# NVlabs/L4P

Measured on AMD Instinct MI355X. Metric: frames/sec (all heads), 16x224x224 clip; encoder MFMA-roofline %, higher is better.
Workload: dtype bf16; 1 GPU; configs[2]: single MI355X, all heads (depth+flow+track2d/3d+motion-seg+pose), bf16, batch=4 clips, 64 track queries per clip; parallelism=dp1 (clips sharded, no collective in the step)

## Files before the change

### l4p_amd/csrc/gemm8p.hpp

```cpp
#pragma once
#include "gemm.hpp"

#ifdef GEMM_PROBE_VARIANTS
static __device__ int g_tile_gm = 0;
#endif
template <int WR, int WC, int TM, int TN>
struct Gemm8pCfg {
    static constexpr int BM = WR * TM * 16, BN = WC * TN * 16;
    static constexpr int A_HALF = WR * TM * 8 * 128, W_HALF = (WC * TN * 8 + 63) / 64 * 64 * 128;
    static constexpr int LDS_BYTES = 2 * (2 * A_HALF + 2 * W_HALF);
};
template <typename T, int MODE, int WR, int WC, bool SPLITK = false, int TM = 8, int TN = 4, bool PERSIST = false, bool SUBPIX = false>
__global__ __launch_bounds__(512) void gemm8p_kernel(const GemmParams p) {
    static_assert(!PERSIST || (MODE == 0 && !SPLITK), "persistent form: dense GEMM without split-K");
    static_assert(!SUBPIX || (MODE == 1 && !SPLITK && !PERSIST), "sub-pixel conv: the conv form without split-K");
    static_assert(WR * WC == 8 && (WC == 2 || WC == 4), "8 waves");
    static_assert(TM % 2 == 0 && TN % 2 == 0 && (WR * TM) % 8 == 0, "half tiles; A half-tile = whole 64-row staging passes");
    constexpr int BM = WR * TM * 16, BN = WC * TN * 16, BK = 64;
    constexpr int RH = TM * 8, CH = TN * 8;
    constexpr int A_PASS = WR * RH / 64, W_PASS = (WC * CH + 63) / 64;
    constexpr int A_HALF = WR * RH * 128, W_HALF = W_PASS * 64 * 128;
    constexpr int BUF = 2 * A_HALF + 2 * W_HALF;
    constexpr int INFLIGHT = 2 * A_PASS + 2 * W_PASS;
    typedef const __attribute__((address_space(1))) void* gptr_t;
    typedef __attribute__((address_space(3))) void* lptr_t;

    extern __shared__ __attribute__((aligned(16))) char smem[];

    const int wave = __builtin_amdgcn_readfirstlane((int)threadIdx.x >> 6);
    const int wr = wave / WC, wc = wave % WC, grp = wave >> 2;
    int li, kg, srow, slot, cs_a, cs_w[W_PASS], a_off[2], w_off[2];
    auto lane_setup = [&](int tid) {
        const int lane = tid & 63;
        li = lane & 15, kg = lane >> 4;
        srow = tid >> 3, slot = tid & 7;
        cs_a = slot ^ ((srow >> 1) & 7);
#pragma unroll
        for (int i = 0; i < W_PASS; ++i) {
            const int lr = srow + 64 * i;
            cs_w[i] = slot ^ (((((lr % CH) / (2 * TN)) & 3) << 1) | ((lr >> 1) & 1));
        }
        const int sw_a = (li >> 1) & 7, sw_w = (((li >> 2) & 3) << 1) | ((li >> 1) & 1);
#pragma unroll
        for (int kk = 0; kk < 2; ++kk) {
            a_off[kk] = (wr * RH + li) * 128 + (((kk * 4 + kg) ^ sw_a) << 4);
            w_off[kk] = (wc * CH + 2 * TN * (li >> 2) + (li & 3)) * 128 + (((kk * 4 + kg) ^ sw_w) << 4);
        }
    };
    lane_setup((int)threadIdx.x);

    const int ntn = (p.N + BN - 1) / BN, ntm = (p.M + BM - 1) / BM, ntiles = ntn * ntm;
    const int nsplit = SPLITK ? p.splitk : 1;
    const int ksplit = SPLITK ? (int)blockIdx.x / ntiles : 0;
    const int bid0 = SPLITK ? (int)blockIdx.x - ksplit * ntiles : (int)blockIdx.x;
    auto decode_tile = [&](int bid, int& m0_, int& n0_) {
        int tile;
        {
            const int xcd = bid & 7, idx = bid >> 3, q = ntiles >> 3, r = ntiles & 7;
            tile = (xcd < r ? xcd * (q + 1) : r * (q + 1) + (xcd - r) * q) + idx;
        }
        int mt, nt_;
        {
            const int nb = (ntn + 7) >> 3, bw = (ntn + nb - 1) / nb, full = (nb - 1) * ntm * bw;
#ifdef GEMM_PROBE_VARIANTS
            const bool banded = g_tile_gm >= 0;
#else
            const bool banded = true;
#endif
            if (!banded || nb == 1) {
                mt = tile / ntn;
                nt_ = tile % ntn;
            } else if (tile < full) {
                const int band = tile / (ntm * bw), rem = tile - band * (ntm * bw);
                mt = rem / bw;
                nt_ = band * bw + rem % bw;
            } else {
                const int w = ntn - (nb - 1) * bw, rem = tile - full;
                mt = rem / w;
                nt_ = (nb - 1) * bw + rem % w;
            }
        }
        if (MODE == 1) mt = conv_tile_walk(p, mt, BM, 2);
        m0_ = mt * BM, n0_ = nt_ * BN;
    };
    int bid = bid0, m0, n0;
    decode_tile(bid, m0, n0);

    const char* a_src[A_PASS][2];
    unsigned a_mask[A_PASS][2];
    const char* w_src[W_PASS][2];
    auto setup_src = [&](int m0, int n0) {
#pragma unroll
    for (int i = 0; i < A_PASS; ++i)
#pragma unroll
        for (int h = 0; h < 2; ++h) {
            const int lra = i * 64 + srow;
            int m = m0 + (lra / RH) * (TM * 16) + h * RH + lra % RH;
// ... 43 lines not shown
    const int kt0 = SPLITK ? (int)((long long)nk_all * ksplit / nsplit) : 0;
    const int nk = SPLITK ? (int)((long long)nk_all * (ksplit + 1) / nsplit) - kt0 : nk_all;
    const char* zero = (const char*)g_zero_chunk;

    struct ConvPos {
        int kt, tap, ci0;
        long long off;
        int bit;
    } cpos[2];
    auto conv_tap_off = [&](int tap) {
        const int dt = tap / 9 - 1, dh = (tap / 3) % 3 - 1, dw = tap % 3 - 1;
        return ((((long long)dt * p.Hi + dh) * p.Wi + dw) * p.Cin) * 2;
    };
    if (MODE == 1) {
#pragma unroll
        for (int h = 0; h < 2; ++h) {
            const int first = SUBPIX ? subpix_tap(cells, 0) : 0;
            cpos[h] = ConvPos{0, 0, 0, conv_tap_off(first), first};
        }
    }
    auto stage_a = [&](int h, int kt, int buf) {
        long long off;
        int tap = 0;
        if (MODE == 0) {
            off = (long long)(kt0 + kt) * (BK * 2);
        } else {
            ConvPos& c = cpos[h];
            while (c.kt < kt0 + kt) {
                ++c.kt;
                c.ci0 += BK;
                if (c.ci0 == p.Cin) {
                    c.ci0 = 0;
                    ++c.tap;
                    if constexpr (SUBPIX) {
                        c.bit = subpix_tap(cells, c.tap);
                        c.off = conv_tap_off(c.bit);
                    } else {
                        c.off = conv_tap_off(c.tap < 27 ? c.tap : 26);
                    }
                }
            }
            tap = SUBPIX ? c.bit : c.tap;
            off = c.off + (long long)c.ci0 * 2;
        }
#pragma unroll
        for (int i = 0; i < A_PASS; ++i) {
            bool ok;
            if (MODE == 0)
                ok = (!SPLITK || kt < nk) && (kt0 + kt) * BK + cs_a * 8 < p.K;
            else
                ok = kt < nk && ((a_mask[i][h] >> tap) & 1u);
            const char* src = ok ? a_src[i][h] + off : zero;
            __builtin_amdgcn_global_load_lds((gptr_t)src, (lptr_t)(smem + buf * BUF + h * A_HALF + (i * 512 + wave * 64) * 16), 16,
                                             0, 0);
        }
    };
    auto stage_w = [&](int h, int kt, int buf) {
#pragma unroll
        for (int i = 0; i < W_PASS; ++i) {
            const bool ok = (!SPLITK || kt < nk) && (kt0 + kt) * BK + cs_w[i] * 8 < p.K && w_src[i][h] != nullptr;
            const char* src = ok ? w_src[i][h] + (long long)(kt0 + kt) * (BK * 2) : zero;
            __builtin_amdgcn_global_load_lds((gptr_t)src,
                                             (lptr_t)(smem + buf * BUF + 2 * A_HALF + h * W_HALF + (i * 512 + wave * 64) * 16), 16, 0, 0);
        }
    };

    f32x4 acc[TM][TN];
    vec8<T> xa[TM / 2][2], wb[2][TN / 2][2];

    auto read_a = [&](int h, int buf) {
        const char* base = smem + buf * BUF + h * A_HALF;
#pragma unroll
        for (int ii = 0; ii < TM / 2; ++ii)
#pragma unroll
            for (int kk = 0; kk < 2; ++kk) xa[ii][kk] = *(const vec8<T>*)(base + a_off[kk] + ii * 2048);
    };
    auto read_w = [&](int h, int buf) {
        const char* base = smem + buf * BUF + 2 * A_HALF + h * W_HALF;
#pragma unroll
        for (int jj = 0; jj < TN / 2; ++jj)
#pragma unroll
            for (int kk = 0; kk < 2; ++kk) wb[h][jj][kk] = *(const vec8<T>*)(base + w_off[kk] + jj * 512);
    };
    auto quadrant = [&](int qa, int qw) {
        __builtin_amdgcn_s_setprio(1);
#pragma unroll
        for (int kk = 0; kk < 2; ++kk)
#pragma unroll
            for (int ii = 0; ii < TM / 2; ++ii)
#pragma unroll
                for (int jj = 0; jj < TN / 2; ++jj)
                    acc[qa * (TM / 2) + ii][qw * (TN / 2) + jj] =
                        mma16(wb[qw][jj][kk], xa[ii][kk], acc[qa * (TM / 2) + ii][qw * (TN / 2) + jj]);
        __builtin_amdgcn_s_setprio(0);
    };
    auto seg_end = [&]() {
        asm volatile("s_waitcnt vmcnt(%0)" ::"n"(INFLIGHT) : "memory");
        __builtin_amdgcn_s_barrier();
        __builtin_amdgcn_sched_barrier(0);
    };
    auto phase_end = [&]() {
        __builtin_amdgcn_sched_barrier(0);
        __builtin_amdgcn_s_barrier();
        __builtin_amdgcn_sched_barrier(0);
    };

    auto prologue_stage = [&]() {
        stage_a(0, 0, 0);
        stage_w(0, 0, 0);
        stage_w(1, 0, 0);
        stage_a(1, 0, 0);
        stage_a(0, 1, 1);
        stage_w(0, 1, 1);
    };
    prologue_stage();
    for (;;) {
    asm volatile("s_waitcnt vmcnt(%0)" ::"n"(INFLIGHT) : "memory");
    __builtin_amdgcn_s_barrier();
    __builtin_amdgcn_sched_barrier(0);
    if (grp == 1) __builtin_amdgcn_s_barrier();
    __builtin_amdgcn_sched_barrier(0);
#pragma unroll
    for (int i = 0; i < TM; ++i)
#pragma unroll
        for (int j = 0; j < TN; ++j) acc[i][j] = (f32x4){0.f, 0.f, 0.f, 0.f};

    auto ktile = [&](int t, auto cur_c) {
        constexpr int cur = decltype(cur_c)::value, nxt = cur ^ 1;
        read_w(0, cur);
        read_a(0, cur);
        stage_w(1, t + 1, nxt);
        seg_end();
        quadrant(0, 0);
        phase_end();
        read_w(1, cur);
        stage_a(1, t + 1, nxt);
        seg_end();
        quadrant(0, 1);
        phase_end();
        read_a(1, cur);
        stage_a(0, t + 2, cur);
        seg_end();
        quadrant(1, 1);
        phase_end();
        stage_w(0, t + 2, cur);
        seg_end();
        quadrant(1, 0);
        phase_end();
    };
    for (int t = 0; t < nk; t += 2) {
        ktile(t, std::integral_constant<int, 0>{});
        if (t + 1 < nk) ktile(t + 1, std::integral_constant<int, 1>{});
    }
    if (grp == 0) __builtin_amdgcn_s_barrier();
    asm volatile("s_waitcnt vmcnt(0)" ::: "memory");

    int nm0 = 0, nn0 = 0;
    bool more = false;
    if constexpr (PERSIST) {
        const int nbid = bid + (int)gridDim.x;
        more = nbid < ntiles;
        if (more) {
            bid = nbid;
            decode_tile(nbid, nm0, nn0);
            setup_src(nm0, nn0);
            prologue_stage();
        }
    }

    if constexpr (SPLITK) {
        const int nb2 = n0 + wc * (TN * 16) + 4 * TN * kg;
#pragma unroll
        for (int i = 0; i < TM; ++i) {
            const int m = m0 + wr * (TM * 16) + i * 16 + li;
            if (m >= p.M) continue;
            float* pp = p.partial + ((long long)ksplit * p.M + m) * p.N + nb2;
#pragma unroll
            for (int j = 0; j < TN; ++j)
                if (nb2 + 4 * j < p.N) *(f32x4*)(pp + 4 * j) = acc[i][j];
        }
        return;
    }
#ifdef GEMM_DBG_NOEPI
#pragma unroll
    for (int i = 0; i < TM; ++i)
#pragma unroll
        for (int j = 0; j < TN; ++j) asm volatile("" ::"v"(acc[i][j]));
#else
#ifdef GEMM_DBG_ONLY_FAST
    gemm_epilogue_dense<T, TM, TN, ACT_NONE, 0>(p, acc, m0 + wr * (TM * 16), n0 + wc * (TN * 16), li, kg);
    return;
#endif
    if constexpr (SUBPIX) {
        gemm_epilogue_subpixel<T, TM, TN>(p, acc, m0 + wr * (TM * 16), n0 + wc * (TN * 16), li, kg);
    } else if (TN == 4 && p.epi == EPI_MASKDOT) {
        if constexpr (TN == 4) gemm_epilogue_maskdot<T, TM, TN>(p, acc, m0 + wr * (TM * 16), n0 + wc * (TN * 16), li, kg);
    } else if (!gemm_epilogue_dense_dispatch<T, TM, TN>(p, acc, m0 + wr * (TM * 16), n0 + wc * (TN * 16), li, kg)) {
        if constexpr (TN == 4) gemm_epilogue<T, TM, TN, true>(p, acc, m0 + wr * (TM * 16), n0 + wc * (TN * 16), li, kg);
    }
#endif
    if constexpr (!PERSIST) {
        break;
    } else {
        if (!more) break;
        m0 = nm0, n0 = nn0;
        asm volatile("" : "+s"(m0), "+s"(n0));
        int t_ = (int)threadIdx.x;
        asm volatile("" : "+v"(t_));
        lane_setup(t_);
        setup_src(m0, n0);
    }
    }
}
```

### l4p_amd/csrc/gemm_launch.hpp

```cpp
#pragma once
#include <cstdlib>
#include <cstring>

#include "gemm.hpp"
#include "gemm8p.hpp"
#ifdef L4P_PROBE_KERNELS
#include "gemm4w.hpp"
#endif
#include "conv3_halo.hpp"
#include "gemm_select.hpp"
#include "gemm_skinny.hpp"
#include "prof.hpp"

template <typename T>
__global__ void splitk_finish_kernel(const GemmParams p) {
    const long long total = (long long)p.M * (p.N / 8);
    for (long long i = blockIdx.x * (long long)blockDim.x + threadIdx.x; i < total; i += (long long)gridDim.x * blockDim.x) {
        const int m = (int)(i / (p.N / 8)), n = (int)(i % (p.N / 8)) * 8;
        float v[8] = {0.f, 0.f, 0.f, 0.f, 0.f, 0.f, 0.f, 0.f};
        for (int s = 0; s < p.splitk; ++s) {
            const float* pp = p.partial + ((long long)s * p.M + m) * p.N + n;
            const f32x4 a = *(const f32x4*)pp, b = *(const f32x4*)(pp + 4);
#pragma unroll
            for (int q = 0; q < 4; ++q) {
                v[q] += a[q];
                v[4 + q] += b[q];
            }
        }
        if (p.bias) {
#pragma unroll
            for (int q = 0; q < 8; ++q) v[q] += p.bias[n + q];
        }
        if (p.act == ACT_GELU) {
#pragma unroll
            for (int q = 0; q < 8; ++q) v[q] = gelu_for<T>(v[q]);
        } else if (p.act == ACT_RELU) {
#pragma unroll
            for (int q = 0; q < 8; ++q) v[q] = fmaxf(v[q], 0.f);
        }
        if (p.res1) {
            const long long roff = (long long)(p.res_mod > 0 ? (m % p.res_mod) : m) * p.ldr + n;
#pragma unroll
            for (int q = 0; q < 8; ++q) {
                v[q] += p.res_f32 ? ((const float*)p.res1)[roff + q] : to_f32<T>(((const T*)p.res1)[roff + q]);
                if (p.res2) v[q] += p.res_f32 ? ((const float*)p.res2)[roff + q] : to_f32<T>(((const T*)p.res2)[roff + q]);
            }
        }
        const long long off = (long long)m * p.ldc + n;
        if (p.out_f32) {
#pragma unroll
            for (int q = 0; q < 8; ++q) p.out_f32[off + q] = v[q];
        }
        if (p.out_T) {
#pragma unroll
            for (int q = 0; q < 8; ++q) ((T*)p.out_T)[off + q] = from_f32<T>(v[q]);
        }
        if (p.out_relu_T) {
#pragma unroll
            for (int q = 0; q < 8; ++q) ((T*)p.out_relu_T)[off + q] = from_f32<T>(fmaxf(v[q], 0.f));
        }
    }
}
template <typename T>
static void launch_splitk_finish(const GemmParams& p, int nsplit, hipStream_t stream) {
    if (nsplit <= 1 || (p.tuning & 2)) return;
    const long long total = (long long)p.M * (p.N / 8);
    const int grid = (int)((total + 255) / 256 < 4096 ? (total + 255) / 256 : 4096);
    hipLaunchKernelGGL(splitk_finish_kernel<T>, dim3(grid), dim3(256), 0, stream, p);
}

static inline ProfScope gemm_prof(int cls, hipStream_t stream, const GemmParams& p, int K, GemmForm form, int nsplit = 1) {
    if (!g_prof_on) return ProfScope(cls, stream);
    char buf[GEMM_TAG_MAX];
    return ProfScope(cls, stream, "M%d N%d K%d epi%d act%d %s", p.M, p.N, K, p.epi, p.act, gemm_form_tag(form, nsplit, buf));
}

template <typename T, int BM, int BN, int MODE, bool GLDS, int STAGES = 2, bool GROUPW = false>
static int launch_cfg(const GemmParams& p, hipStream_t stream, GemmForm form) {
    constexpr int WM = 2, WN = 2;
    const int ntm = (p.M + BM - 1) / BM, ntn = (p.N + BN - 1) / BN;
    const int nsplit = p.splitk > 1 ? p.splitk : 1;
    const size_t lds = STAGES * (BM + BN) * 128;
    auto kern = gemm_kernel<T, BM, BN, WM, WN, MODE, GLDS, STAGES, GROUPW>;
    static lds_attr_state attr_done;
    HIP_TRY(lds_attr_once(attr_done, kern, (int)lds));
    ProfScope prof = gemm_prof(MODE == 0 ? (p.w_gr > 0 || p.M < 1024 ? PROF_GEMM_SMALL : PROF_GEMM) : PROF_CONV3D, stream, p, p.K, form, nsplit);
    hipLaunchKernelGGL(kern, dim3(ntm * ntn * nsplit), dim3(WM * WN * 64), lds, stream, p);
    launch_splitk_finish<T>(p, nsplit, stream);
    HIP_TRY(hipGetLastError());
    return 0;
}

template <typename T>
static int launch_subpixel(const GemmParams& p, hipStream_t stream, GemmForm form) {
    constexpr int BM = 128, BN = 128;
    const int ntm = (p.M + BM - 1) / BM, ntn = p.N / BN;
    const size_t lds = 2 * (BM + BN) * 128;
    auto kern = gemm_kernel<T, BM, BN, 2, 2, 1, true, 2, false, true>;
    static lds_attr_state attr_done;
    HIP_TRY(lds_attr_once(attr_done, kern, (int)lds));
    ProfScope prof = gemm_prof(PROF_CONV3D, stream, p, subpixel_mean_k(p), form);
    hipLaunchKernelGGL(kern, dim3(ntm * ntn), dim3(256), lds, stream, p);
    HIP_TRY(hipGetLastError());
    return 0;
}

template <typename T, int MODE, int WR, int WC, bool SPLITK = false, int TM = 8, int TN = 4>
static int launch_8p(const GemmParams& p, hipStream_t stream, GemmForm form) {
    typedef Gemm8pCfg<WR, WC, TM, TN> Cfg;
    const int ntm = (p.M + Cfg::BM - 1) / Cfg::BM, ntn = (p.N + Cfg::BN - 1) / Cfg::BN;
    const int nsplit = SPLITK ? p.splitk : 1;
    const size_t lds = Cfg::LDS_BYTES;
    auto kern = gemm8p_kernel<T, MODE, WR, WC, SPLITK, TM, TN, false>;
    static lds_attr_state attr_done;
    HIP_TRY(lds_attr_once(attr_done, kern, (int)lds));
    ProfScope prof = gemm_prof(MODE == 0 ? PROF_GEMM : PROF_CONV3D, stream, p, p.K, form, nsplit);
    hipLaunchKernelGGL(kern, dim3(ntm * ntn * nsplit), dim3(512), lds, stream, p);
    launch_splitk_finish<T>(p, nsplit, stream);
    HIP_TRY(hipGetLastError());
    return 0;
}
template <typename T>
static int launch_8p_subpixel(const GemmParams& p, hipStream_t stream, GemmForm form) {
    typedef Gemm8pCfg<2, 4, 8, 4> Cfg;
    const int ntm = (p.M + Cfg::BM - 1) / Cfg::BM, ntn = p.N / Cfg::BN;
    auto kern = gemm8p_kernel<T, 1, 2, 4, false, 8, 4, false, true>;
    static lds_attr_state attr_done;
    HIP_TRY(lds_attr_once(attr_done, kern, (int)Cfg::LDS_BYTES));
    ProfScope prof = gemm_prof(PROF_CONV3D, stream, p, subpixel_mean_k(p), form);
    hipLaunchKernelGGL(kern, dim3(ntm * ntn), dim3(512), Cfg::LDS_BYTES, stream, p);
    HIP_TRY(hipGetLastError());
    return 0;
}

#ifdef L4P_PROBE_KERNELS
template <typename T, bool SPLITK>
static int launch_4w(const GemmParams& p, hipStream_t stream, GemmForm form) {
    typedef Gemm4wCfg Cfg;
    const int ntm = (p.M + Cfg::BM - 1) / Cfg::BM, ntn = (p.N + Cfg::BN - 1) / Cfg::BN;
    const int nsplit = SPLITK ? p.splitk : 1;
    auto kern = gemm4w_kernel<T, SPLITK>;
    static lds_attr_state attr_done;
    HIP_TRY(lds_attr_once(attr_done, kern, Cfg::LDS_BYTES));
    ProfScope prof = gemm_prof(PROF_GEMM, stream, p, p.K, form, nsplit);
    hipLaunchKernelGGL(kern, dim3(ntm * ntn * nsplit), dim3(256), Cfg::LDS_BYTES, stream, p);
    launch_splitk_finish<T>(p, nsplit, stream);
    HIP_TRY(hipGetLastError());
    return 0;
}
#endif

template <typename T, int WR, int WC, bool UPS = false, bool TWO_PHASE = UPS>
static int launch_halo(const GemmParams& p, hipStream_t stream, GemmForm form) {
    typedef ConvHaloCfg<WR, WC> Cfg;
    typedef ConvHaloTile<WR, WC> Tile;
    static_assert(Cfg::BM == Tile::BM && Cfg::BN == Tile::BN && Cfg::TT == Tile::TT && Cfg::TH == Tile::TH && Cfg::TW == Tile::TW, "gemm_select.hpp");
    static_assert(TWO_PHASE || !UPS, "the fused up-sampling loader exists on the two-phase body only");
    auto kern = TWO_PHASE ? conv3_halo2p_kernel<T, WR, WC, UPS> : conv3_halo_kernel<T, WR, WC, false>;
    static lds_attr_state attr_done;
    HIP_TRY(lds_attr_once(attr_done, kern, Cfg::LDS_BYTES));
    ProfScope prof = gemm_prof(PROF_CONV3D, stream, p, p.K, form);
    hipLaunchKernelGGL(kern, dim3(p.M / Cfg::BM), dim3(512), Cfg::LDS_BYTES, stream, p);
    HIP_TRY(hipGetLastError());
    return 0;
}

template <typename T, bool GROUPW>
static int launch_skinny(const GemmParams& p, hipStream_t stream, GemmForm form) {
    const int grid = ((p.M + 15) / 16) * ((p.N + 31) / 32);
    ProfScope prof = gemm_prof(PROF_GEMM_SMALL, stream, p, p.K, form);
    hipLaunchKernelGGL((gemm_skinny_kernel<T, GROUPW>), dim3(grid), dim3(64), 0, stream, p);
    HIP_TRY(hipGetLastError());
    return 0;
}

static GemmKnobs gemm_knobs() {
    GemmKnobs k;
    k.gemm_variant = knob(KNOB_GEMM_VARIANT), k.conv_halo = knob(KNOB_CONV_HALO), k.gemm_skinny = knob(KNOB_GEMM_SKINNY);
    k.skinny_max_m = knob(KNOB_SKINNY_MAX_M), k.gemm_deep = knob(KNOB_GEMM_DEEP), k.gemm_group = knob(KNOB_GEMM_GROUP);
    k.track_deep = knob(KNOB_TRACK_DEEP), k.gemm_t192 = knob(KNOB_GEMM_T192), k.gemm_4w = knob(KNOB_GEMM_4W);
#ifdef L4P_PROBE_KERNELS
    k.probe_kernels = 1;
#else
    k.probe_kernels = 0;
#endif
    return k;
}

template <typename T>
static int launch_form(GemmForm form, const GemmParams& p, hipStream_t stream) {
    switch (form) {
        case GEMM_STAGED_128x64: return launch_cfg<T, 128, 64, 0, true>(p, stream, form);
        case GEMM_STAGED_128x64_DEEP: return launch_cfg<T, 128, 64, 0, true, 4>(p, stream, form);
        case GEMM_STAGED_128x128: return launch_cfg<T, 128, 128, 0, true>(p, stream, form);
        case GEMM_WGRP_128x64: return launch_cfg<T, 128, 64, 0, true, 2, true>(p, stream, form);
        case GEMM_WGRP_128x128: return launch_cfg<T, 128, 128, 0, true, 2, true>(p, stream, form);
        case GEMM_CONV_128x64: return launch_cfg<T, 128, 64, 1, true>(p, stream, form);
        case GEMM_CONV_128x128: return launch_cfg<T, 128, 128, 1, true>(p, stream, form);
        case GEMM_CONV_RELU_128x64: return launch_cfg<T, 128, 64, 1, false>(p, stream, form);
        case GEMM_CONV_RELU_128x128: return launch_cfg<T, 128, 128, 1, false>(p, stream, form);
        case GEMM_SUBPIX_STAGED: return launch_subpixel<T>(p, stream, form);
        default: break;
    }
    if constexpr (sizeof(T) == 2) {
        switch (form) {
            case GEMM_WGRP_64x64_DEEP: return launch_cfg<T, 64, 64, 0, true, 4, true>(p, stream, form);
            case GEMM_WGRP_128x64_DEEP: return launch_cfg<T, 128, 64, 0, true, 4, true>(p, stream, form);
            case GEMM_8P_256x256: return launch_8p<T, 0, 2, 4>(p, stream, form);
            case GEMM_8P_256x192: return launch_8p<T, 0, 4, 2, false, 4, 6>(p, stream, form);
            case GEMM_8P_SK_256x256: return launch_8p<T, 0, 2, 4, true>(p, stream, form);
            case GEMM_8P_SK_256x192: return launch_8p<T, 0, 4, 2, true, 4, 6>(p, stream, form);
            case GEMM_8P_CONV: return launch_8p<T, 1, 2, 4>(p, stream, form);
            case GEMM_HALO_2x4: return launch_halo<T, 2, 4>(p, stream, form);
            case GEMM_HALO_4x2: return launch_halo<T, 4, 2>(p, stream, form);
            case GEMM_HALO_2x4_2P: return launch_halo<T, 2, 4, false, true>(p, stream, form);
            case GEMM_HALO_4x2_2P: return launch_halo<T, 4, 2, false, true>(p, stream, form);
            case GEMM_SKINNY: return launch_skinny<T, false>(p, stream, form);
            case GEMM_SKINNY_WGRP: return launch_skinny<T, true>(p, stream, form);
            case GEMM_SUBPIX_8P: return launch_8p_subpixel<T>(p, stream, form);
#ifdef L4P_PROBE_KERNELS
            case GEMM_HALO_4x2_UPS: return launch_halo<T, 4, 2, true>(p, stream, form);
            case GEMM_4W: return launch_4w<T, false>(p, stream, form);
#endif
            default: break;
        }
    }
    l4p_set_error("gemm: kernel form %d does not exist for this element type in this build", (int)form);
    return L4P_E_INVALID;
}

template <typename T>
int launch_gemm_typed(int mode, const GemmParams& p_in, hipStream_t stream) {
    const int epi_generic = knob(KNOB_EPI_GENERIC);
    const bool maskdot_valu = p_in.epi == L4P_EPI_MASKDOT && !knob(KNOB_MASKDOT_MFMA);
    GemmParams patched;
    const GemmParams* p = &p_in;
    if (epi_generic || maskdot_valu) {
        patched = p_in;
        if (epi_generic) patched.tuning |= 1;
        if (maskdot_valu) patched.tuning |= 4;
        p = &patched;
    }
    const char* err = nullptr;
    const GemmForm form = gemm_select(mode, (int)sizeof(T), *p, gemm_knobs(), &err);
    if (form == GEMM_FORM_INVALID) {
        l4p_set_error("%s", err);
        return L4P_E_INVALID;
    }
    return launch_form<T>(form, *p, stream);
}

static int fill_group(GemmGroupParams& g, const GemmParams* p, int n, int bm, int bn) {
    std::memset(&g, 0, sizeof(g));
    int first = 0;
    for (int i = 0; i < L4P_GEMM_GROUP_MAX; ++i) {
        g.first[i] = first;
        if (i < n) {
            g.p[i] = p[i];
            first += ((p[i].M + bm - 1) / bm) * ((p[i].N + bn - 1) / bn);
        } else {
            g.first[i] = 0x7FFFFFFF;
        }
    }
    g.first[L4P_GEMM_GROUP_MAX] = first;
    return first;
}

template <typename T>
int launch_gemm_group_typed(const GemmParams* p, int n, hipStream_t stream) {
    static_assert(sizeof(T) == 2, "the grouped kernels exist for the 16-bit types");
    const char* err = nullptr;
    const GemmGroupForm form = gemm_group_select(p, n, gemm_knobs(), &err);
    if (form == GEMM_GROUP_INVALID) {
        l4p_set_error("%s", err);
        return L4P_E_INVALID;
    }
    if (form == GEMM_GROUP_ONE_BY_ONE) {
        for (int i = 0; i < n; ++i) {
            const int rc = launch_gemm_typed<T>(0, p[i], stream);
            if (rc) return rc;
        }
        return 0;
    }
    GemmGroupParams g;
    if (form == GEMM_GROUP_SKINNY) {
        const int grid = fill_group(g, p, n, 16, 32);
        ProfScope prof(PROF_GEMM_SMALL, stream, "group of %d: M%d N%d K%d ... %s", n, p[0].M, p[0].N, p[0].K, gemm_group_tag(form));
        hipLaunchKernelGGL(gemm_skinny_group_kernel<T>, dim3(grid), dim3(64), 0, stream, g);
        HIP_TRY(hipGetLastError());
        return 0;
    }
    const int grid = fill_group(g, p, n, 128, 64);
// ... 11 lines not shown
```

### l4p_amd/csrc/gemm_select.hpp

```cpp
#pragma once
#include <cstdio>

#include "l4p_hip.h"

enum GemmForm {
    GEMM_FORM_INVALID = 0,
    GEMM_STAGED_128x64,
    GEMM_STAGED_128x64_DEEP,
    GEMM_STAGED_128x128,
    GEMM_WGRP_64x64_DEEP,
    GEMM_WGRP_128x64_DEEP,
    GEMM_WGRP_128x64,
    GEMM_WGRP_128x128,
    GEMM_CONV_128x64,
    GEMM_CONV_128x128,
    GEMM_CONV_RELU_128x64,
    GEMM_CONV_RELU_128x128,
    GEMM_8P_256x256,
    GEMM_8P_256x192,
    GEMM_8P_SK_256x256,
    GEMM_8P_SK_256x192,
    GEMM_8P_CONV,
    GEMM_HALO_2x4,
    GEMM_HALO_4x2,
    GEMM_HALO_2x4_2P,
    GEMM_HALO_4x2_2P,
    GEMM_HALO_4x2_UPS,
    GEMM_SKINNY,
    GEMM_SKINNY_WGRP,
    GEMM_4W,
    GEMM_SUBPIX_STAGED,
    GEMM_SUBPIX_8P,
    GEMM_FORM_NUM
};

enum GemmGroupForm { GEMM_GROUP_INVALID = 0, GEMM_GROUP_SKINNY, GEMM_GROUP_DEEP, GEMM_GROUP_ONE_BY_ONE };

struct GemmKnobs {
    int gemm_variant, conv_halo, gemm_skinny, skinny_max_m, gemm_deep, gemm_group, track_deep, gemm_t192, gemm_4w;
    int probe_kernels;
};

enum { GEMM_TAG_MAX = 40 };
inline const char* gemm_form_tag(GemmForm form, int nsplit, char (&buf)[GEMM_TAG_MAX]) {
    const char* head = "";
    const char* tail = nullptr;
    switch (form) {
        case GEMM_STAGED_128x64: tail = " t128x64"; break;
        case GEMM_STAGED_128x64_DEEP: tail = " t128x64 deep"; break;
        case GEMM_STAGED_128x128: tail = " t128x128"; break;
        case GEMM_WGRP_64x64_DEEP: tail = " t64x64 deep wgrp"; break;
        case GEMM_WGRP_128x64_DEEP: tail = " t128x64 deep wgrp"; break;
        case GEMM_WGRP_128x64: tail = " t128x64 wgrp"; break;
        case GEMM_WGRP_128x128: tail = " t128x128 wgrp"; break;
        case GEMM_CONV_128x64: tail = " t128x64"; break;
        case GEMM_CONV_128x128: tail = " t128x128"; break;
        case GEMM_CONV_RELU_128x64: tail = " t128x64"; break;
        case GEMM_CONV_RELU_128x128: tail = " t128x128"; break;
        case GEMM_8P_SK_256x256: head = "8p ", tail = " t256x256"; break;
        case GEMM_8P_SK_256x192: head = "8p ", tail = " t256x192"; break;
        case GEMM_8P_256x256: return "8p t256x256";
        case GEMM_8P_256x192: return "8p t256x192";
        case GEMM_8P_CONV: return "8p t256x256";
        case GEMM_HALO_2x4: return "halo t256x256";
        case GEMM_HALO_4x2: return "halo t512x128";
        case GEMM_HALO_2x4_2P: return "halo 2p t256x256";
        case GEMM_HALO_4x2_2P: return "halo 2p t512x128";
        case GEMM_HALO_4x2_UPS: return "halo ups t512x128";
        case GEMM_SKINNY: return "skinny";
        case GEMM_SKINNY_WGRP: return "wgrp skinny";
        case GEMM_4W: return "4w t256x128";
        case GEMM_SUBPIX_STAGED: return "subpix t128x128";
        case GEMM_SUBPIX_8P: return "subpix 8p t256x256";
        default: return "invalid";
    }
    snprintf(buf, sizeof buf, "%ssk%d%s", head, nsplit, tail);
    return buf;
}
inline const char* gemm_group_tag(GemmGroupForm form) { return form == GEMM_GROUP_SKINNY ? "skinny" : form == GEMM_GROUP_DEEP ? "t128x64 deep" : "one by one"; }

inline long long gemm_tiles(const l4p_gemm_desc& p, int bm, int bn) { return (long long)((p.M + bm - 1) / bm) * ((p.N + bn - 1) / bn); }

inline bool gemm_is_big(const l4p_gemm_desc& p) {
    const long long t128 = gemm_tiles(p, 128, 128);
    return (t128 >= 400 && !(t128 > 512 && t128 < 640)) || (p.splitk > 1 && p.N >= 256);
}

inline bool gemm_is_small_deep(const l4p_gemm_desc& p) {
    return !gemm_is_big(p) && p.splitk <= 1 && !p.relu_in && gemm_tiles(p, 128, 64) <= 256 && p.K >= 6 * 64 && !(p.tuning & 1) && p.w_gr == 0;
}

inline bool gemm_is_skinny(const l4p_gemm_desc& p, const GemmKnobs& k) {
    return k.gemm_skinny && p.M >= 1 && p.M <= k.skinny_max_m && p.K >= 64 && p.K % 64 == 0 && p.lda % 8 == 0 && p.ldw % 8 == 0 && p.N % 8 == 0 &&
           p.w_gr == 0 && p.kw_cols == 0 && p.splitk <= 1 && !p.relu_in && p.epi == L4P_EPI_DENSE && !(p.tuning & 4) &&
           gemm_tiles(p, 16, 32) <= 512;
}
inline bool gemm_is_skinny_grouped(const l4p_gemm_desc& p, const GemmKnobs& k) {
    return k.gemm_skinny && p.w_gr > 0 && p.w_gr % 16 == 0 && p.M >= 1 && p.M <= 2048 && p.K >= 64 && p.K % 64 == 0 && p.lda % 8 == 0 &&
           p.ldw % 8 == 0 && p.N % 8 == 0 && p.a_gr == 0 && p.splitk <= 1 && !p.relu_in && p.epi == L4P_EPI_DENSE && !(p.tuning & 4) &&
           gemm_tiles(p, 16, 32) <= 512;
}

inline bool dense_epilogue_is_lean(const l4p_gemm_desc& p) {
    if ((p.tuning & 1) || p.epi != L4P_EPI_DENSE || p.res_mod > 0 || p.c_gr > 0 || p.a_gr > 0) return false;
    const int res = !p.res1 ? 0 : (p.res_f32 ? 1 : 2);
    if (res == 1 && p.res2) return false;
    return (res == 0) || (res == 1 && p.act == L4P_ACT_NONE) || (res == 2 && (p.act == L4P_ACT_NONE || p.act == L4P_ACT_RELU));
}
inline bool epilogue_is_lean_8p(const l4p_gemm_desc& p) {
    if (p.tuning & 1) return false;
    if (p.epi == L4P_EPI_QKV) return !p.res1 && p.act == L4P_ACT_NONE && p.c_gr == 0;
    if (p.epi == L4P_EPI_CONVT) return !p.res1 && p.act == L4P_ACT_NONE && p.out_T && !p.out_f32 && !p.out_relu_T;
    return dense_epilogue_is_lean(p);
}

template <int WR, int WC>
struct ConvHaloTile {
    static constexpr int BM = WR * 128, BN = WC * 64;
    static constexpr int TT = 2, TW = 16, TH = BM / (TT * TW);
};
template <int WR, int WC>
inline bool conv_halo_fits(const l4p_gemm_desc& p) {
    typedef ConvHaloTile<WR, WC> Cfg;
    if (p.ups_hi > 0 && !(WR == 4 && WC == 2 && p.ups_wi > 0 && (long long)p.ups_hi * p.ups_wi * p.Cin * 2 < (1ll << 31))) return false;
    return p.N == Cfg::BN && p.st == 1 && p.sh == 1 && p.sw == 1 && p.Cin % 32 == 0 && p.To % Cfg::TT == 0 && p.Ho % Cfg::TH == 0 &&
           p.Wo % Cfg::TW == 0 && p.To == p.Ti && p.Ho == p.Hi && p.Wo == p.Wi && p.M / Cfg::BM >= 192 && p.ldc == p.N &&
           (!p.res1 || p.ldr == p.N) && (long long)p.M * p.Cin * 2 < (1ll << 32) && !p.relu_in && p.splitk <= 1 && dense_epilogue_is_lean(p);
}

inline bool gemm4w_fits(const l4p_gemm_desc& p) {
    if (p.relu_in || p.K % 8 || p.N <= 128) return false;
    const long long pm = p.a_gr > 0 ? (long long)((p.M - 1) / p.a_gr) * p.a_gs + p.a_go + p.a_gr : p.M;
    return pm * p.lda * 2 < (1ll << 31) && (long long)p.N * p.ldw * 2 < (1ll << 31);
}

inline bool kw_cols_ok(int mode, const l4p_gemm_desc& p, const char** err) {
    if (mode != 0 || p.w_gr > 0 || p.splitk > 1 || p.relu_in || p.kw_cols % 128 || p.kw_len < 1 || p.K % 8) {
        *err = "l4p_gemm: kw_cols needs a dense GEMM without split-K / row groups, kw_cols a multiple of 128";
        return false;
    }
    return true;
}

inline int subpixel_mean_k(const l4p_gemm_desc& p, int* min_cells_out = nullptr) {
    int cells = 0, min_cells = 27;
    for (int s = 0; s < p.kt * p.kh * p.kw; ++s) {
        const int ks[3] = {p.kt, p.kh, p.kw}, ss[3] = {s / (p.kw * p.kh), (s / p.kw) % p.kh, s % p.kw};
        int n = 1;
        for (int a = 0; a < 3; ++a) n *= ks[a] == 1 ? 3 : (ss[a] == 0 || ss[a] == ks[a] - 1) ? 2 : 1;
        cells += n;
        min_cells = n < min_cells ? n : min_cells;
    }
    if (min_cells_out) *min_cells_out = min_cells;
    return (int)((long long)cells * p.Cin / (p.kt * p.kh * p.kw));
}

inline GemmForm gemm_select(int mode, int esize, const l4p_gemm_desc& p, const GemmKnobs& k, const char** err) {
    const bool t16 = esize == 2;
    const int variant = k.gemm_variant;
    if (mode == 2) {
        int min_cells;
        subpixel_mean_k(p, &min_cells);
        const long long t8 = (long long)((p.M + 255) / 256) * (p.N / 256);
        if (t16 && p.Cout % 256 == 0 && p.Cin % 64 == 0 && min_cells * (p.Cin / 64) >= 2 && variant != 1 && (variant == 10 || t8 >= 256))
            return GEMM_SUBPIX_8P;
        return GEMM_SUBPIX_STAGED;
    }
    if (p.kw_cols > 0) {
        if (!kw_cols_ok(mode, p, err)) return GEMM_FORM_INVALID;
        return t16 && gemm_tiles(p, 128, 64) <= 256 ? GEMM_STAGED_128x64_DEEP : GEMM_STAGED_128x64;
    }
    if (p.w_gr > 0) {
        if (mode != 0 || p.splitk > 1 || p.relu_in || p.w_gr % 128 || p.K % 8) {
            *err = "l4p_gemm: row-grouped weights need a dense GEMM without split-K, w_gr a multiple of 128";
            return GEMM_FORM_INVALID;
        }
        if (t16) {
            if (gemm_is_skinny_grouped(p, k)) return GEMM_SKINNY_WGRP;
            if (k.track_deep && p.N <= 64 && (long long)((p.M + 127) / 128) <= 256 && p.K >= 6 * 64) {
                return (p.M + 127) / 128 <= 128 && p.w_gr % 64 == 0 ? GEMM_WGRP_64x64_DEEP : GEMM_WGRP_128x64_DEEP;
            }
        }
        return p.N <= 64 ? GEMM_WGRP_128x64 : GEMM_WGRP_128x128;
    }
    if (t16 && mode == 0 && gemm_is_skinny(p, k)) return GEMM_SKINNY;
    const bool big = gemm_is_big(p);
    if (t16) {
        if (mode == 1 && p.ups_hi > 0) {
            if (!k.probe_kernels) {
                *err = "conv3d: the fused up-sampling loader (l4p_gemm_desc.ups_hi) is a measured-and-not-adopted form: build with PROBES=1";
                return GEMM_FORM_INVALID;
            }
            if (conv_halo_fits<4, 2>(p)) return GEMM_HALO_4x2_UPS;
            *err = "conv3d: the fused up-sampling loader takes N == 128, stride 1, Cin % 32 == 0, whole 2 x 16 x 16 output blocks";
            return GEMM_FORM_INVALID;
        }
        if (mode == 1 && k.conv_halo && variant != 1) {
            if (conv_halo_fits<2, 4>(p)) return k.conv_halo == 2 ? GEMM_HALO_2x4_2P : GEMM_HALO_2x4;
            if (conv_halo_fits<4, 2>(p)) return k.conv_halo == 2 ? GEMM_HALO_4x2_2P : GEMM_HALO_4x2;
        }
        if (p.splitk > 1 && mode == 0 && !p.relu_in && p.K % 8 == 0 && variant != 1 && p.N > 128) {
            const long long w8 = gemm_tiles(p, 256, 256) * p.splitk;
            const long long w192 = gemm_tiles(p, 256, 192) * p.splitk;
            if (k.gemm_t192 && w192 > w8 && w192 <= 256 && w8 >= 144 && p.K / p.splitk >= 512) return GEMM_8P_SK_256x192;
            if (w8 >= 144 && w8 <= 256 && p.K / p.splitk >= 512) return GEMM_8P_SK_256x256;
        }
        if (p.splitk <= 1 && !p.relu_in && p.K % 8 == 0 && variant != 1 && p.N > 128) {
            const long long t8 = gemm_tiles(p, 256, 256);
            const bool use8 = variant == 10 || (variant == 0 && (t8 >= 256 || (t8 >= 192 && p.M >= 4096) || (t8 >= 144 && p.K >= 1024)));
            if (use8 && mode == 0) {
                if (k.probe_kernels && k.gemm_4w) {
                    const long long t4 = gemm_tiles(p, 256, 128);
                    const bool pays = t4 >= 512 && (p.epi == L4P_EPI_MASKDOT || p.K <= 512 || (p.epi == L4P_EPI_QKV && t4 >= 1024));
                    if (gemm4w_fits(p) && (k.gemm_4w >= 2 || pays)) return GEMM_4W;
                }
                const long long n192 = gemm_tiles(p, 256, 192);
                const long long c256 = (t8 + 255) / 256 * 65536, c192 = (n192 + 255) / 256 * 49152;
                return k.gemm_t192 && c192 < c256 && epilogue_is_lean_8p(p) ? GEMM_8P_256x192 : GEMM_8P_256x256;
            }
            if (use8 && mode == 1 && p.Cin % 64 == 0) return GEMM_8P_CONV;
        }
    }
    if (mode == 0) {
        if (variant == 3) return GEMM_STAGED_128x64;
        if (t16 && !big && p.splitk <= 1 && k.gemm_deep && gemm_tiles(p, 128, 64) <= 256 && p.K >= 6 * 64) return GEMM_STAGED_128x64_DEEP;
        return big ? GEMM_STAGED_128x128 : GEMM_STAGED_128x64;
    }
    if (p.relu_in) return big ? GEMM_CONV_RELU_128x128 : GEMM_CONV_RELU_128x64;
    return big ? GEMM_CONV_128x128 : GEMM_CONV_128x64;
}

inline GemmGroupForm gemm_group_select(const l4p_gemm_desc* p, int n, const GemmKnobs& k, const char** err) {
    for (int i = 0; i < n; ++i)
        if (p[i].kw_cols > 0 && !kw_cols_ok(0, p[i], err)) return GEMM_GROUP_INVALID;
    if (!k.gemm_group || n < 2 || n > L4P_GEMM_GROUP_MAX) return GEMM_GROUP_ONE_BY_ONE;
    bool sk = true;
    long long waves = 0;
    for (int i = 0; sk && i < n; ++i) {
        sk = gemm_is_skinny(p[i], k);
        waves += gemm_tiles(p[i], 16, 32);
    }
    if (sk && waves <= 1024) return GEMM_GROUP_SKINNY;
    bool ok = k.gemm_deep != 0;
    long long total = 0;
    for (int i = 0; ok && i < n; ++i) {
        ok = gemm_is_small_deep(p[i]);
        total += gemm_tiles(p[i], 128, 64);
    }
    return ok && total <= 512 ? GEMM_GROUP_DEEP : GEMM_GROUP_ONE_BY_ONE;
}
```

### l4p_amd/csrc/prof.hip

```cpp
#include "prof.hpp"

#include <algorithm>
#include <atomic>
#include <cstdlib>
#include <cstring>
#include <map>
#include <mutex>
#include <string>
#include <vector>

#include "common.hpp"

bool g_prof_on = false;

namespace {
struct KnobDef {
    const char* name;
    const char* env;
    int dflt;
};
const KnobDef kKnobs[KNOB_NUM] = {{"conv_halo", "L4P_CONV_HALO", 1}, {"gemm_4w", "L4P_GEMM_4W", 0},
                                   {"maskdot_mfma", "L4P_MASKDOT_MFMA", 1},
                                   {"conv_ups", "L4P_CONV_UPS", 0},
                                   {"ln_tracks", "L4P_LN_TRACKS", 1},
                                   {"ln_rows16", "L4P_LN_ROWS16", 1},
                                   {"attn64", "L4P_ATTN64", 1},
                                   {"gemm_skinny", "L4P_GEMM_SKINNY", 1},
                                   {"readout_wide", "L4P_READOUT_WIDE", 1},
                                   {"track_deep", "L4P_TRACK_DEEP", 1},
                                   {"track_fold_l0", "L4P_TRACK_FOLD_L0", 1},
                                   {"track_fold_t2i", "L4P_TRACK_FOLD_T2I", 1},
                                   {"track_fold_t2i_v", "L4P_TRACK_FOLD_T2I_V", 1},
                                   {"track_kwin", "L4P_TRACK_KWIN", 1},
                                   {"track_ln_chain", "L4P_TRACK_LN_CHAIN", 1},
                                   {"track_fold_i2t", "L4P_TRACK_FOLD_I2T", 1},
                                   {"track_fold_pair", "L4P_TRACK_FOLD_PAIR", 0},
                                   {"track_delta_kernel", "L4P_TRACK_DELTA_KERNEL", 1},
                                   {"gemm_persist", "L4P_GEMM_PERSIST", 1},
                                   {"skinny_max_m", "L4P_SKINNY_MAX_M", 128},
                                   {"gemm_deep", "L4P_GEMM_DEEP", 1},
                                   {"gemm_group", "L4P_GEMM_GROUP", 1},
                                   {"epi_generic", "L4P_EPI_GENERIC", 0},
                                   {"gemm_variant", "L4P_GEMM_VARIANT", 0},
                                   {"gemm_t192", "L4P_GEMM_T192", 1},
                                   {"attn_persist", "L4P_ATTN_PERSIST", 1},
                                   {"attn_variant", "L4P_ATTN_VARIANT", 0},
                                   {"ups_ipt", "L4P_UPS_IPT", 2},
                                   {"ups_nt", "L4P_UPS_NT", 1},
                                   {"fc2_splitk8", "L4P_FC2_SPLITK8", -1},
                                   {"enc_defer_res", "L4P_ENC_DEFER_RES", 1},
                                   {"enc_sk_in_ln", "L4P_ENC_SK_IN_LN", 1},
                                   {"dpt_fold_rn", "L4P_DPT_FOLD_RN", 1},
                                   {"probe_kernels", "", 0}};
std::atomic<int> g_knob[KNOB_NUM];
std::once_flag g_knob_once;
#ifdef L4P_PROBE_KERNELS
constexpr bool kProbeKernels = true;
#else
constexpr bool kProbeKernels = false;
#endif
bool probe_only(int i) { return i == KNOB_GEMM_4W || i == KNOB_CONV_UPS; }
void knobs_init() {
    for (int i = 0; i < KNOB_NUM; ++i) {
        const char* e = kKnobs[i].env[0] ? getenv(kKnobs[i].env) : nullptr;
        int v = e ? atoi(e) : kKnobs[i].dflt;
        if (i == KNOB_PROBE_KERNELS) v = kProbeKernels ? 1 : 0;
        if (probe_only(i) && !kProbeKernels) v = 0;
        g_knob[i].store(v, std::memory_order_relaxed);
    }
}
}
int knob(int id) {
    std::call_once(g_knob_once, knobs_init);
    return g_knob[id].load(std::memory_order_relaxed);
}

namespace {
struct Pair {
    hipEvent_t a, b;
    int cls;
    char tag[64];
};
std::mutex g_mu;
std::vector<Pair> g_pairs;
std::vector<hipEvent_t> g_pool;
const char* kNames[PROF_NUM] = {"gemm", "conv3d", "attention", "layernorm", "elementwise", "track", "preprocess", "gemm_small"};

hipEvent_t get_event() {
    if (!g_pool.empty()) {
        hipEvent_t e = g_pool.back();
        g_pool.pop_back();
        return e;
    }
    hipEvent_t e;
    (void)hipEventCreate(&e);
    return e;
}
}

void prof_begin(int cls, hipStream_t stream, const char* tag) {
    std::lock_guard<std::mutex> lk(g_mu);
    Pair p{get_event(), get_event(), cls, {0}};
    if (tag) snprintf(p.tag, sizeof p.tag, "%s", tag);
    (void)hipEventRecord(p.a, stream);
    g_pairs.push_back(p);
}
void prof_end(int cls, hipStream_t stream) {
    std::lock_guard<std::mutex> lk(g_mu);
    for (size_t i = g_pairs.size(); i-- > 0;)
        if (g_pairs[i].cls == cls) {
            (void)hipEventRecord(g_pairs[i].b, stream);
            return;
        }
}

extern "C" {
int l4p_set_knob(const char* name, int value) {
    std::call_once(g_knob_once, knobs_init);
    for (int i = 0; i < KNOB_NUM; ++i)
        if (name && !strcmp(name, kKnobs[i].name)) {
            if (i == KNOB_PROBE_KERNELS || (probe_only(i) && !kProbeKernels && value != 0)) {
                l4p_set_error("l4p_set_knob: '%s' %s", name, i == KNOB_PROBE_KERNELS ? "is read-only (1 in a PROBES=1 build of the library)"
                                                                                       : "selects a kernel this build does not contain (make PROBES=1)");
                return L4P_E_INVALID;
            }
            g_knob[i].store(value, std::memory_order_relaxed);
            return L4P_OK;
// ... 68 lines not shown
```

### l4p_amd/csrc/prof.hpp

```cpp
#pragma once
#include <hip/hip_runtime.h>

#include <cstdarg>
#include <cstdio>

enum ProfClass {
    PROF_GEMM = 0,
    PROF_CONV3D,
    PROF_ATTENTION,
    PROF_LAYERNORM,
    PROF_ELEMENTWISE,
    PROF_TRACK,
    PROF_PREP,
    PROF_GEMM_SMALL,
    PROF_NUM
};

enum Knob {
    KNOB_CONV_HALO = 0, KNOB_GEMM_4W, KNOB_MASKDOT_MFMA, KNOB_CONV_UPS, KNOB_LN_TRACKS, KNOB_LN_ROWS16, KNOB_ATTN64, KNOB_GEMM_SKINNY,
    KNOB_READOUT_WIDE, KNOB_TRACK_DEEP,
    KNOB_TRACK_FOLD_L0, KNOB_TRACK_FOLD_T2I, KNOB_TRACK_FOLD_T2I_V, KNOB_TRACK_KWIN, KNOB_TRACK_LN_CHAIN, KNOB_TRACK_FOLD_I2T,
    KNOB_TRACK_FOLD_PAIR, KNOB_TRACK_DELTA_KERNEL,
    KNOB_GEMM_PERSIST, KNOB_SKINNY_MAX_M, KNOB_GEMM_DEEP, KNOB_GEMM_GROUP, KNOB_EPI_GENERIC, KNOB_GEMM_VARIANT, KNOB_GEMM_T192,
    KNOB_ATTN_PERSIST, KNOB_ATTN_VARIANT, KNOB_UPS_IPT, KNOB_UPS_NT, KNOB_FC2_SPLITK8, KNOB_ENC_DEFER_RES, KNOB_ENC_SK_IN_LN,
    KNOB_DPT_FOLD_RN,
    KNOB_PROBE_KERNELS, KNOB_NUM
};
int knob(int id);

void prof_begin(int cls, hipStream_t stream, const char* tag = nullptr);
void prof_end(int cls, hipStream_t stream);
extern bool g_prof_on;

struct ProfScope {
    int cls;
    hipStream_t s;
    ProfScope(int c, hipStream_t st) : cls(c), s(st) {
        if (g_prof_on) prof_begin(cls, s);
    }
    ProfScope(int c, hipStream_t st, const char* fmt, ...) __attribute__((format(printf, 4, 5))) : cls(c), s(st) {
        if (!g_prof_on) return;
        char tag[64];
        va_list ap;
        va_start(ap, fmt);
        vsnprintf(tag, sizeof tag, fmt, ap);
        va_end(ap);
        prof_begin(cls, s, tag);
    }
    ~ProfScope() {
        if (g_prof_on) prof_end(cls, s);
    }
};
```

Before: 1024 frames/s.

## Add two-phase 8-wave GEMM body with hoisted tail checks for deep K

Adds a TWOPH variant of the 8-wave ping-pong GEMM that merges the four per-k-tile barrier segments into two. Each segment runs two MFMA quadrants and issues its prefetch loads in batches. The variant also stages an extra W half in the prologue, pre-advances source pointers, and runs the steady-state loop with K-tail bounds checks compiled out, keeping them only for the final tiles. By default it is selected for the 256x256 and 256x192 dense forms when K >= 512, with a knob to force either body. The aim is to cut barrier and waitcnt overhead per k-tile. In exchange it holds more fragments in registers and lowers load/compute interleaving granularity, with extra complexity in the pointer-stepping logic.

Measured after the change: 1047 frames/s, median of 6. 1.02x the previous value.

```diff
diff --git a/l4p_amd/csrc/gemm8p.hpp b/l4p_amd/csrc/gemm8p.hpp
--- a/l4p_amd/csrc/gemm8p.hpp
+++ b/l4p_amd/csrc/gemm8p.hpp
@@ -10,9 +10,11 @@
     static constexpr int A_HALF = WR * TM * 8 * 128, W_HALF = (WC * TN * 8 + 63) / 64 * 64 * 128;
     static constexpr int LDS_BYTES = 2 * (2 * A_HALF + 2 * W_HALF);
 };
-template <typename T, int MODE, int WR, int WC, bool SPLITK = false, int TM = 8, int TN = 4, bool PERSIST = false, bool SUBPIX = false>
+template <typename T, int MODE, int WR, int WC, bool SPLITK = false, int TM = 8, int TN = 4, bool PERSIST = false, bool SUBPIX = false,
+          bool TWOPH = false>
 __global__ __launch_bounds__(512) void gemm8p_kernel(const GemmParams p) {
     static_assert(!PERSIST || (MODE == 0 && !SPLITK), "persistent form: dense GEMM without split-K");
+    static_assert(!TWOPH || (MODE == 0 && !SPLITK && !PERSIST), "two-phase body: dense GEMM without split-K, one tile per workgroup");
     static_assert(!SUBPIX || (MODE == 1 && !SPLITK && !PERSIST), "sub-pixel conv: the conv form without split-K");
     static_assert(WR * WC == 8 && (WC == 2 || WC == 4), "8 waves");
     static_assert(TM % 2 == 0 && TN % 2 == 0 && (WR * TM) % 8 == 0, "half tiles; A half-tile = whole 64-row staging passes");
@@ -222,8 +224,7 @@
 #pragma unroll
             for (int kk = 0; kk < 2; ++kk) wb[h][jj][kk] = *(const vec8<T>*)(base + w_off[kk] + jj * 512);
     };
-    auto quadrant = [&](int qa, int qw) {
-        __builtin_amdgcn_s_setprio(1);
+    auto quadrant_mfma = [&](int qa, int qw) {
 #pragma unroll
         for (int kk = 0; kk < 2; ++kk)
 #pragma unroll
@@ -232,6 +233,10 @@
                 for (int jj = 0; jj < TN / 2; ++jj)
                     acc[qa * (TM / 2) + ii][qw * (TN / 2) + jj] =
                         mma16(wb[qw][jj][kk], xa[ii][kk], acc[qa * (TM / 2) + ii][qw * (TN / 2) + jj]);
+    };
+    auto quadrant = [&](int qa, int qw) {
+        __builtin_amdgcn_s_setprio(1);
+        quadrant_mfma(qa, qw);
         __builtin_amdgcn_s_setprio(0);
     };
     auto seg_end = [&]() {
@@ -252,8 +257,50 @@
         stage_a(1, 0, 0);
         stage_a(0, 1, 1);
         stage_w(0, 1, 1);
+        if constexpr (TWOPH) stage_w(1, 1, 1);
     };
     prologue_stage();
+
+    constexpr bool W_FILL = (WC * CH) % 64 != 0;
+    int w_step_last = BK * 2;
+    if constexpr (TWOPH) {
+#pragma unroll
+        for (int i = 0; i < A_PASS; ++i) {
+            a_src[i][0] += 2 * BK * 2;
+            a_src[i][1] += BK * 2;
+        }
+#pragma unroll
+        for (int i = 0; i < W_PASS; ++i)
+#pragma unroll
+            for (int h = 0; h < 2; ++h) w_src[i][h] = w_src[i][h] != nullptr ? w_src[i][h] + 2 * BK * 2 : zero;
+        if (W_FILL && srow + 64 * (W_PASS - 1) >= WC * CH) w_step_last = 0;
+    }
+    auto stage_a2 = [&](auto tail_c, int h, int kt, int buf) {
+#pragma unroll
+        for (int i = 0; i < A_PASS; ++i) {
+            const char* src = a_src[i][h];
+            if constexpr (decltype(tail_c)::value) src = kt * BK + cs_a * 8 < p.K ? src : zero;
+            __builtin_amdgcn_global_load_lds((gptr_t)src, (lptr_t)(smem + buf * BUF + h * A_HALF + (i * 512 + wave * 64) * 16), 16,
+                                             0, 0);
+            a_src[i][h] += BK * 2;
+        }
+    };
+    auto stage_w2 = [&](auto tail_c, int h, int kt, int buf) {
+#pragma unroll
+        for (int i = 0; i < W_PASS; ++i) {
+            const char* src = w_src[i][h];
+            if constexpr (decltype(tail_c)::value) src = kt * BK + cs_w[i] * 8 < p.K ? src : zero;
+            __builtin_amdgcn_global_load_lds((gptr_t)src,
+                                             (lptr_t)(smem + buf * BUF + 2 * A_HALF + h * W_HALF + (i * 512 + wave * 64) * 16), 16, 0, 0);
+            w_src[i][h] += (W_FILL && i == W_PASS - 1) ? w_step_last : BK * 2;
+        }
+    };
+    auto seg_end2 = [&]() {
+        __builtin_amdgcn_sched_barrier(0);
+        asm volatile("s_waitcnt vmcnt(%0) lgkmcnt(0)" ::"n"(INFLIGHT) : "memory");
+        __builtin_amdgcn_s_barrier();
+        __builtin_amdgcn_sched_barrier(0);
+    };
     for (;;) {
     asm volatile("s_waitcnt vmcnt(%0)" ::"n"(INFLIGHT) : "memory");
     __builtin_amdgcn_s_barrier();
@@ -288,9 +335,46 @@
         quadrant(1, 0);
         phase_end();
     };
-    for (int t = 0; t < nk; t += 2) {
-        ktile(t, std::integral_constant<int, 0>{});
-        if (t + 1 < nk) ktile(t + 1, std::integral_constant<int, 1>{});
+    auto ktile2 = [&](int t, auto cur_c, auto tail_c) {
+        constexpr int cur = decltype(cur_c)::value, nxt = cur ^ 1;
+        read_w(0, cur);
+        read_w(1, cur);
+        read_a(0, cur);
+        stage_a2(tail_c, 1, t + 1, nxt);
+        seg_end2();
+        __builtin_amdgcn_s_setprio(1);
+        quadrant_mfma(0, 0);
+        quadrant_mfma(0, 1);
+        __builtin_amdgcn_s_setprio(0);
+        phase_end();
+        read_a(1, cur);
+        stage_a2(tail_c, 0, t + 2, cur);
+        stage_w2(tail_c, 0, t + 2, cur);
+        stage_w2(tail_c, 1, t + 2, cur);
+        seg_end2();
+        __builtin_amdgcn_s_setprio(1);
+        quadrant_mfma(1, 1);
+        quadrant_mfma(1, 0);
+        __builtin_amdgcn_s_setprio(0);
+        phase_end();
+    };
+    if constexpr (TWOPH) {
+        const std::integral_constant<int, 0> b0{};
+        const std::integral_constant<int, 1> b1{};
+        int t = 0;
+        for (const int nfull = p.K / BK; t + 3 < nfull; t += 2) {
+            ktile2(t, b0, std::false_type{});
+            ktile2(t + 1, b1, std::false_type{});
+        }
+        for (; t < nk; t += 2) {
+            ktile2(t, b0, std::true_type{});
+            if (t + 1 < nk) ktile2(t + 1, b1, std::true_type{});
+        }
+    } else {
+        for (int t = 0; t < nk; t += 2) {
+            ktile(t, std::integral_constant<int, 0>{});
+            if (t + 1 < nk) ktile(t + 1, std::integral_constant<int, 1>{});
+        }
     }
     if (grp == 0) __builtin_amdgcn_s_barrier();
     asm volatile("s_waitcnt vmcnt(0)" ::: "memory");
diff --git a/l4p_amd/csrc/gemm_launch.hpp b/l4p_amd/csrc/gemm_launch.hpp
--- a/l4p_amd/csrc/gemm_launch.hpp
+++ b/l4p_amd/csrc/gemm_launch.hpp
@@ -105,13 +105,13 @@
     return 0;
 }
 
-template <typename T, int MODE, int WR, int WC, bool SPLITK = false, int TM = 8, int TN = 4>
+template <typename T, int MODE, int WR, int WC, bool SPLITK = false, int TM = 8, int TN = 4, bool TWOPH = false>
 static int launch_8p(const GemmParams& p, hipStream_t stream, GemmForm form) {
     typedef Gemm8pCfg<WR, WC, TM, TN> Cfg;
     const int ntm = (p.M + Cfg::BM - 1) / Cfg::BM, ntn = (p.N + Cfg::BN - 1) / Cfg::BN;
     const int nsplit = SPLITK ? p.splitk : 1;
     const size_t lds = Cfg::LDS_BYTES;
-    auto kern = gemm8p_kernel<T, MODE, WR, WC, SPLITK, TM, TN, false>;
+    auto kern = gemm8p_kernel<T, MODE, WR, WC, SPLITK, TM, TN, false, false, TWOPH>;
     static lds_attr_state attr_done;
     HIP_TRY(lds_attr_once(attr_done, kern, (int)lds));
     ProfScope prof = gemm_prof(MODE == 0 ? PROF_GEMM : PROF_CONV3D, stream, p, p.K, form, nsplit);
@@ -184,6 +184,7 @@
 #else
     k.probe_kernels = 0;
 #endif
+    k.gemm_8p_body = knob(KNOB_GEMM_8P_BODY);
     return k;
 }
 
@@ -206,8 +207,15 @@
         switch (form) {
             case GEMM_WGRP_64x64_DEEP: return launch_cfg<T, 64, 64, 0, true, 4, true>(p, stream, form);
             case GEMM_WGRP_128x64_DEEP: return launch_cfg<T, 128, 64, 0, true, 4, true>(p, stream, form);
-            case GEMM_8P_256x256: return launch_8p<T, 0, 2, 4>(p, stream, form);
-            case GEMM_8P_256x192: return launch_8p<T, 0, 4, 2, false, 4, 6>(p, stream, form);
+            case GEMM_8P_256x256:
+                return gemm_8p_two_phase(p, form) ? launch_8p<T, 0, 2, 4, false, 8, 4, true>(p, stream, form) : launch_8p<T, 0, 2, 4>(p, stream, form);
+            case GEMM_8P_256x192:
+                return gemm_8p_two_phase(p, form) ? launch_8p<T, 0, 4, 2, false, 4, 6, true>(p, stream, form)
+                                                  : launch_8p<T, 0, 4, 2, false, 4, 6>(p, stream, form);
+            case GEMM_8P_2PH_256x256: return launch_8p<T, 0, 2, 4, false, 8, 4, true>(p, stream, form);
+            case GEMM_8P_2PH_256x192: return launch_8p<T, 0, 4, 2, false, 4, 6, true>(p, stream, form);
+            case GEMM_8P_4PH_256x256: return launch_8p<T, 0, 2, 4>(p, stream, form);
+            case GEMM_8P_4PH_256x192: return launch_8p<T, 0, 4, 2, false, 4, 6>(p, stream, form);
             case GEMM_8P_SK_256x256: return launch_8p<T, 0, 2, 4, true>(p, stream, form);
             case GEMM_8P_SK_256x192: return launch_8p<T, 0, 4, 2, true, 4, 6>(p, stream, form);
             case GEMM_8P_CONV: return launch_8p<T, 1, 2, 4>(p, stream, form);
diff --git a/l4p_amd/csrc/gemm_select.hpp b/l4p_amd/csrc/gemm_select.hpp
--- a/l4p_amd/csrc/gemm_select.hpp
+++ b/l4p_amd/csrc/gemm_select.hpp
@@ -31,6 +31,10 @@
     GEMM_4W,
     GEMM_SUBPIX_STAGED,
     GEMM_SUBPIX_8P,
+    GEMM_8P_2PH_256x256,
+    GEMM_8P_2PH_256x192,
+    GEMM_8P_4PH_256x256,
+    GEMM_8P_4PH_256x192,
     GEMM_FORM_NUM
 };
 
@@ -39,6 +43,7 @@
 struct GemmKnobs {
     int gemm_variant, conv_halo, gemm_skinny, skinny_max_m, gemm_deep, gemm_group, track_deep, gemm_t192, gemm_4w;
     int probe_kernels;
+    int gemm_8p_body;
 };
 
 enum { GEMM_TAG_MAX = 40 };
@@ -72,6 +77,10 @@
         case GEMM_4W: return "4w t256x128";
         case GEMM_SUBPIX_STAGED: return "subpix t128x128";
         case GEMM_SUBPIX_8P: return "subpix 8p t256x256";
+        case GEMM_8P_2PH_256x256: return "8p 2ph t256x256";
+        case GEMM_8P_2PH_256x192: return "8p 2ph t256x192";
+        case GEMM_8P_4PH_256x256: return "8p 4ph t256x256";
+        case GEMM_8P_4PH_256x192: return "8p 4ph t256x192";
         default: return "invalid";
     }
     snprintf(buf, sizeof buf, "%ssk%d%s", head, nsplit, tail);
@@ -112,6 +121,10 @@
     if (p.epi == L4P_EPI_QKV) return !p.res1 && p.act == L4P_ACT_NONE && p.c_gr == 0;
     if (p.epi == L4P_EPI_CONVT) return !p.res1 && p.act == L4P_ACT_NONE && p.out_T && !p.out_f32 && !p.out_relu_T;
     return dense_epilogue_is_lean(p);
+}
+
+inline bool gemm_8p_two_phase(const l4p_gemm_desc& p, GemmForm form) {
+    return (form == GEMM_8P_256x256 || form == GEMM_8P_256x192) && p.K >= 8 * 64;
 }
 
 template <int WR, int WC>
@@ -216,7 +229,10 @@
                 }
                 const long long n192 = gemm_tiles(p, 256, 192);
                 const long long c256 = (t8 + 255) / 256 * 65536, c192 = (n192 + 255) / 256 * 49152;
-                return k.gemm_t192 && c192 < c256 && epilogue_is_lean_8p(p) ? GEMM_8P_256x192 : GEMM_8P_256x256;
+                const bool t192 = k.gemm_t192 && c192 < c256 && epilogue_is_lean_8p(p);
+                if (k.gemm_8p_body == 1) return t192 ? GEMM_8P_2PH_256x192 : GEMM_8P_2PH_256x256;
+                if (k.gemm_8p_body == 2) return t192 ? GEMM_8P_4PH_256x192 : GEMM_8P_4PH_256x256;
+                return t192 ? GEMM_8P_256x192 : GEMM_8P_256x256;
             }
             if (use8 && mode == 1 && p.Cin % 64 == 0) return GEMM_8P_CONV;
         }
diff --git a/l4p_amd/csrc/prof.hip b/l4p_amd/csrc/prof.hip
--- a/l4p_amd/csrc/prof.hip
+++ b/l4p_amd/csrc/prof.hip
@@ -43,6 +43,7 @@
                                    {"epi_generic", "L4P_EPI_GENERIC", 0},
                                    {"gemm_variant", "L4P_GEMM_VARIANT", 0},
                                    {"gemm_t192", "L4P_GEMM_T192", 1},
+                                   {"gemm_8p_body", "L4P_GEMM_8P_BODY", 0},
                                    {"attn_persist", "L4P_ATTN_PERSIST", 1},
                                    {"attn_variant", "L4P_ATTN_VARIANT", 0},
                                    {"ups_ipt", "L4P_UPS_IPT", 2},
diff --git a/l4p_amd/csrc/prof.hpp b/l4p_amd/csrc/prof.hpp
--- a/l4p_amd/csrc/prof.hpp
+++ b/l4p_amd/csrc/prof.hpp
@@ -22,6 +22,7 @@
     KNOB_TRACK_FOLD_L0, KNOB_TRACK_FOLD_T2I, KNOB_TRACK_FOLD_T2I_V, KNOB_TRACK_KWIN, KNOB_TRACK_LN_CHAIN, KNOB_TRACK_FOLD_I2T,
     KNOB_TRACK_FOLD_PAIR, KNOB_TRACK_DELTA_KERNEL,
     KNOB_GEMM_PERSIST, KNOB_SKINNY_MAX_M, KNOB_GEMM_DEEP, KNOB_GEMM_GROUP, KNOB_EPI_GENERIC, KNOB_GEMM_VARIANT, KNOB_GEMM_T192,
+    KNOB_GEMM_8P_BODY,
     KNOB_ATTN_PERSIST, KNOB_ATTN_VARIANT, KNOB_UPS_IPT, KNOB_UPS_NT, KNOB_FC2_SPLITK8, KNOB_ENC_DEFER_RES, KNOB_ENC_SK_IN_LN,
     KNOB_DPT_FOLD_RN,
     KNOB_PROBE_KERNELS, KNOB_NUM
```
